# r4dl/StopThePop-Rasterization

Measured on AMD Instinct MI355X. Metric: fwd+bwd frames/sec at 1920×1080, 1M Gaussians; PSNR vs reference, higher is better.
Workload: dtype f32

## Files before the change

### stopthepop-rasterization_amd/csrc/stp_binning.hip

```cpp
#include <cstdlib>
#include <cstring>
#include <rocprim/rocprim.hpp>

#include "stp_internal.h"
#include "stp_device.h"

namespace stp {

uint32_t higher_msb(uint32_t n)
{
    uint32_t msb = sizeof(n) * 4, step = msb;
    while (step > 1) {
        step /= 2;
        if (n >> msb) msb += step; else msb -= step;
    }
    if (n >> msb) msb++;
    return msb;
}

size_t scan_temp_bytes(size_t P)
{
    size_t bytes = 0;
    (void)rocprim::inclusive_scan(nullptr, bytes, (uint32_t*)nullptr, (uint32_t*)nullptr, P, rocprim::plus<uint32_t>());
    return bytes;
}

#include <rocprim/rocprim_version.hpp>
#if ROCPRIM_VERSION_MAJOR == 4 && ROCPRIM_VERSION_MINOR == 2
#define STP_OWN_ONESWEEP 1
#else
#define STP_OWN_ONESWEEP 0
#warning "stp_binning.hip: the own onesweep driver is written against rocPRIM 4.2; with this rocPRIM the tile-bit sort uses rocprim::radix_sort_pairs (check rocprim::detail::onesweep_* against this version, then extend the #if)"
#endif
namespace {
#if STP_OWN_ONESWEEP
namespace rpd = rocprim::detail;
using OsConfig = rpd::wrapped_radix_sort_onesweep_config<rocprim::default_config, uint64_t, uint32_t>;
constexpr rpd::radix_sort_onesweep_config_params os_params()
{
    rpd::radix_sort_onesweep_config_params p = OsConfig::architecture_config<rpd::target_arch::gfx950>::params;
    p.sort.items_per_thread = 8;
#ifdef STP_OS_SORT_BLOCK
    p.sort.block_size = STP_OS_SORT_BLOCK;
#endif
#ifdef STP_OS_SORT_IPT
    p.sort.items_per_thread = STP_OS_SORT_IPT;
#endif
#ifdef STP_OS_HIST_BLOCK
    p.histogram.block_size = STP_OS_HIST_BLOCK;
#endif
#ifdef STP_OS_HIST_IPT
    p.histogram.items_per_thread = STP_OS_HIST_IPT;
#endif
    return p;
}
constexpr rpd::radix_sort_onesweep_config_params OS = os_params();
constexpr unsigned OS_RADIX = 1u << OS.radix_bits_per_place;
constexpr unsigned OS_HIST_ITEMS = OS.histogram.block_size * OS.histogram.items_per_thread;
constexpr unsigned OS_SORT_ITEMS = OS.sort.block_size * OS.sort.items_per_thread;
constexpr unsigned OS_MAX_PLACES = 4;
using OsBlockId = rpd::block_id_wrapper<unsigned int, true>;

struct OsLayout {
    uint32_t* offsets;
    unsigned int* block_ids;
    rpd::onesweep_lookback_state* lookback;
    uint32_t* offsets_tmp;
    uint64_t* keys_tmp;
    uint32_t* values_tmp;
    size_t zero_bytes, total, lookback_offset;
    uint32_t sort_blocks;
};
OsLayout os_layout(char* base, size_t R)
{
    OsLayout L{};
    auto up = [](size_t v) { return (v + 255) & ~(size_t)255; };
    L.sort_blocks = (uint32_t)((R + OS_SORT_ITEMS - 1) / OS_SORT_ITEMS);
    size_t off = 0;
    L.offsets = reinterpret_cast<uint32_t*>(base + off); off += up(sizeof(uint32_t) * OS_MAX_PLACES * OS_RADIX);
    L.block_ids = reinterpret_cast<unsigned int*>(base + off); off += up(sizeof(unsigned int) * OS_MAX_PLACES);
    L.lookback = reinterpret_cast<rpd::onesweep_lookback_state*>(base + off);
    L.lookback_offset = off;
    off += up(sizeof(rpd::onesweep_lookback_state) * OS_MAX_PLACES * OS_RADIX * (size_t)L.sort_blocks);
    L.zero_bytes = off;
    L.offsets_tmp = reinterpret_cast<uint32_t*>(base + off); off += up(sizeof(uint32_t) * OS_RADIX);
    L.keys_tmp = reinterpret_cast<uint64_t*>(base + off); off += up(sizeof(uint64_t) * R);
    L.values_tmp = reinterpret_cast<uint32_t*>(base + off); off += up(sizeof(uint32_t) * R);
    L.total = off;
    return L;
}

__global__ void __launch_bounds__(OS.histogram.block_size) os_histograms_kernel(const uint64_t* keys, uint32_t* counts, uint32_t size, uint32_t full_blocks, unsigned begin_bit, unsigned end_bit)
{
    rpd::onesweep_histograms<OS.histogram.block_size, OS.histogram.items_per_thread, OS.radix_bits_per_place, false>(
        keys, counts, size, full_blocks, rocprim::identity_decomposer{}, begin_bit, end_bit);
}
__global__ void __launch_bounds__(OS.histogram.block_size) os_scan_histograms_kernel(uint32_t* offsets)
{
    rpd::onesweep_scan_histograms<OS.histogram.block_size, OS.radix_bits_per_place>(offsets);
}
__global__ void __launch_bounds__(OS.sort.block_size) os_iteration_kernel(const uint64_t* keys_in, uint64_t* keys_out, const uint32_t* values_in, uint32_t* values_out, unsigned size,
                                                                         uint32_t* offsets_in, uint32_t* offsets_out, rpd::onesweep_lookback_state* lookback, unsigned bit,
                                                                         unsigned radix_bits, unsigned full_blocks, OsBlockId ordered_bid)
{
    rpd::onesweep_iteration<OS.sort.block_size, OS.sort.items_per_thread, OS.radix_bits_per_place, false, OS.radix_rank_algorithm>(
        keys_in, keys_out, values_in, values_out, size, offsets_in, offsets_out, lookback, rocprim::identity_decomposer{}, bit, radix_bits, full_blocks, ordered_bid);
}

constexpr uint32_t OWN_MIN = 1u << 16, OWN_MAX = 1u << 30;
bool own_onesweep_driver(size_t R)
{
    const bool lib = switches().tile_sort == Switches::TILE_SORT_ROCPRIM;
    const bool always = switches().tile_sort == Switches::TILE_SORT_OWN;
    return !lib && (R >= OWN_MIN || (always && R > 0)) && R < OWN_MAX;
}
#else
struct OsLayout { size_t total; };
OsLayout os_layout(char*, size_t) { return OsLayout{0}; }
bool own_onesweep_driver(size_t) { return false; }
#endif
}

size_t sort_temp_bytes(size_t R)
{
    size_t bytes = 0;
    (void)rocprim::radix_sort_pairs(nullptr, bytes, (uint64_t*)nullptr, (uint64_t*)nullptr, (uint32_t*)nullptr, (uint32_t*)nullptr,
                                    R, 0u, 64u);
    const size_t own = os_layout(nullptr, R).total;
    return bytes > own ? bytes : own;
}

void sort_zero_region(const BinningState& b, size_t R, uint32_t tiles, uint32_t** ptr, size_t* words)
{
    *ptr = nullptr; *words = 0;
    if (!own_onesweep_driver(R)) return;
#if STP_OWN_ONESWEEP
    const OsLayout L = os_layout(b.sort_temp, R);
    const uint32_t bit = higher_msb(tiles);
    const size_t places = (bit + OS.radix_bits_per_place - 1) / OS.radix_bits_per_place;
    const size_t bytes = L.lookback_offset + ((sizeof(rpd::onesweep_lookback_state) * places * OS_RADIX * (size_t)L.sort_blocks + 255) & ~(size_t)255);
    *ptr = reinterpret_cast<uint32_t*>(b.sort_temp);
    *words = (bytes < L.zero_bytes ? bytes : L.zero_bytes) / sizeof(uint32_t);
#else
    (void)b; (void)tiles;
#endif
}

hipError_t launch_scan(const FrameParams& f, const GeometryState& g, hipStream_t st)
{
    size_t bytes = g.scan_temp_bytes;
    return rocprim::inclusive_scan(g.scan_temp, bytes, g.tiles_touched, g.point_offsets, (size_t)f.P, rocprim::plus<uint32_t>(), st);
}

hipError_t launch_sort(const FrameParams& f, const BinningState& b, int R, bool tile_bits_only, bool zeroed, hipStream_t st)
{
    if (R <= 0) return hipSuccess;
    const uint32_t bit = higher_msb((uint32_t)(f.gx * f.gy));
    if (!(tile_bits_only && zeroed && own_onesweep_driver((size_t)R))) {
        size_t bytes = b.sort_temp_bytes;
        return rocprim::radix_sort_pairs(b.sort_temp, bytes, b.keys_unsorted, b.keys, b.point_list_unsorted, b.point_list, (size_t)R,
                                         tile_bits_only ? 32u : 0u, 32u + bit, st);
    }
#if STP_OWN_ONESWEEP
    const OsLayout L = os_layout(b.sort_temp, (size_t)R);
    const unsigned begin_bit = 32u, end_bit = 32u + bit;
    const unsigned places = (bit + OS.radix_bits_per_place - 1) / OS.radix_bits_per_place;
    const uint32_t size = (uint32_t)R;
    {
        const uint32_t blocks = (size + OS_HIST_ITEMS - 1) / OS_HIST_ITEMS, full_blocks = size % OS_HIST_ITEMS == 0 ? blocks : blocks - 1;
        hipLaunchKernelGGL(os_histograms_kernel, dim3(blocks), dim3(OS.histogram.block_size), 0, st, b.keys_unsorted, L.offsets, size, full_blocks, begin_bit, end_bit);
        hipLaunchKernelGGL(os_scan_histograms_kernel, dim3(places), dim3(OS.histogram.block_size), 0, st, L.offsets);
    }
    const uint32_t blocks = L.sort_blocks, full_blocks = size % OS_SORT_ITEMS == 0 ? blocks : blocks - 1;
    bool to_output = (places - 1) % 2 == 0, from_input = true;
    for (unsigned place = 0, pbit = begin_bit; place < places; place++, pbit += OS.radix_bits_per_place) {
        const uint64_t* kin = from_input ? b.keys_unsorted : (to_output ? L.keys_tmp : b.keys);
        const uint32_t* vin = from_input ? b.point_list_unsorted : (to_output ? L.values_tmp : b.point_list);
        uint64_t* kout = to_output ? b.keys : L.keys_tmp;
        uint32_t* vout = to_output ? b.point_list : L.values_tmp;
        const unsigned radix_bits = end_bit - pbit < OS.radix_bits_per_place ? end_bit - pbit : OS.radix_bits_per_place;
        hipLaunchKernelGGL(os_iteration_kernel, dim3(blocks), dim3(OS.sort.block_size), 0, st, kin, kout, vin, vout, size, L.offsets + place * OS_RADIX, L.offsets_tmp,
                           L.lookback + (size_t)place * OS_RADIX * blocks, pbit, radix_bits, full_blocks, OsBlockId::create(L.block_ids + place));
        from_input = false;
        to_output = !to_output;
    }
#endif
    return hipGetLastError();
}

namespace {

constexpr int SCAN_THREADS = 1024;

__global__ void __launch_bounds__(SCAN_THREADS) tile_scan_kernel(int tile0, int T, const uint32_t* __restrict__ counts_, uint2* __restrict__ ranges_,
                                                                 uint32_t* __restrict__ cursor_, uint32_t* __restrict__ total)
{
    const uint32_t* __restrict__ counts = counts_ + tile0;
    uint2* __restrict__ ranges = ranges_ + tile0;
    uint32_t* __restrict__ cursor = cursor_ + tile0;
    __shared__ uint32_t s_part[SCAN_THREADS];
    const int tid = (int)threadIdx.x;
    const int per = (T + SCAN_THREADS - 1) / SCAN_THREADS;
    const int lo = min(tid * per, T), hi = min(lo + per, T);
    uint32_t sum = 0;
    for (int t = lo; t < hi; t++) sum += counts[t];
    s_part[tid] = sum;
    __syncthreads();
    for (int off = 1; off < SCAN_THREADS; off <<= 1) {
        const uint32_t v = tid >= off ? s_part[tid - off] : 0u;
        __syncthreads();
        s_part[tid] += v;
        __syncthreads();
    }
    uint32_t run = s_part[tid] - sum;
    for (int t = lo; t < hi; t++) {
        const uint32_t c = counts[t];
        ranges[t] = c ? make_uint2(run, run + c) : make_uint2(0u, 0u);
        cursor[t] = run;
        run += c;
    }
    if (tid == SCAN_THREADS - 1) total[0] = s_part[tid];
}

__global__ void __launch_bounds__(256) bin_pad_kernel(int R, const uint32_t* __restrict__ total, uint64_t* __restrict__ keys, uint32_t* __restrict__ list)
{
    for (int i = (int)total[0] + (int)threadIdx.x; i < R; i += 256) {
        keys[i] = make_sort_key(INVALID_TILE_ID, FLT_MAX);
        list[i] = 0xFFFFFFFFu;
    }
}

}

hipError_t launch_tile_scan(const FrameParams& f, const ImageState& img, hipStream_t st)
{
    hipLaunchKernelGGL(tile_scan_kernel, dim3(1), dim3(SCAN_THREADS), 0, st, f.gx * f.ty0, f.gx * (f.ty1 - f.ty0), img.tile_counts, img.ranges, img.tile_cursor, img.bin_total);
    return hipGetLastError();
}

hipError_t launch_bin_pad(const BinningState& b, const ImageState& img, int R, hipStream_t st)
{
    if (R <= 0) return hipSuccess;
    hipLaunchKernelGGL(bin_pad_kernel, dim3(1), dim3(256), 0, st, R, img.bin_total, b.keys, b.point_list);
    return hipGetLastError();
}

}
```

### stopthepop-rasterization_amd/csrc/stp_forward.hip

```cpp
#include "stp_internal.h"

#include <atomic>
#include <cstring>
#include <mutex>
#include <string>

using namespace stp;

namespace {
struct Mailbox { volatile uint32_t* host = nullptr; uint32_t* dev = nullptr; hipEvent_t ev = nullptr; hipEvent_t done = nullptr; int device = 0; uint32_t ticket = 0; };
constexpr int MAILBOX_RING = 8;
struct MailboxRing { Mailbox slot[MAILBOX_RING]; std::atomic<unsigned> next{0}; std::atomic<bool> ready{false};
                     uint32_t* log_need = nullptr;  };
MailboxRing g_mailboxes[MAX_DEVICES];
std::mutex g_mailbox_mutex;
constexpr int GUESS_SLOTS = 16;
struct SizeGuess { std::atomic<uint64_t> key{0}; std::atomic<uint32_t> R{0}; std::atomic<uint32_t> log_need{0}; };
SizeGuess g_guess[MAX_DEVICES][GUESS_SLOTS];
uint64_t guess_key(const FrameParams& f)
{
    uint64_t k = 0x9E3779B97F4A7C15ull;
    for (uint64_t v : {(uint64_t)f.P, (uint64_t)f.W, (uint64_t)f.H, (uint64_t)f.ty0, (uint64_t)f.ty1, (uint64_t)f.s.sort_mode,
                       (uint64_t)(f.s.tile_based_culling * 8 + f.s.rect_bounding * 4 + f.s.tight_opacity_bounding * 2 + (f.s.sort_order == ORDER_PTD_MAX))})
        k = (k ^ v) * 0xBF58476D1CE4E5B9ull, k ^= k >> 29;
// ... 84 lines not shown
    SideStream* side = nullptr;
    bool colour_started = true;
    char* bin_ptr = nullptr; size_t bin_have = 0;
    uint32_t cap = 0; bool ahead = false, run_ahead = false;
    int* radii; float* const out_color;
    struct Split { const ForwardSplit s; hipStream_t st; bool recorded; ~Split() { if (s.armed && !recorded) (void)hipEventRecord(s.event, st); } } split;
    SideJoin colours;

    ForwardCall(hipStream_t stream, int debug_, const ForwardSplit& split_, int* radii_, float* out_color_)
        : st(stream), debug(debug_), radii(radii_), out_color(out_color_), split{split_, stream, false}, colours{nullptr, stream, false} {}
    int carve_geometry_and_image(stp_alloc_fn geometry_alloc, void* geometry_user, stp_alloc_fn image_alloc, void* image_user, bool with_inv, bool with_stash);
    int launch_up_to_mailbox(); int colour_on_side();
    int request_binning(stp_alloc_fn binning_alloc, void* binning_user);
    int wait_mailbox(); int read_mailbox(int* R_out, bool* wild_out);
    int binning_and_render(const GeometryState& gd, const BinningState& b, int L, uint32_t dup_cap);
};

int ForwardCall::carve_geometry_and_image(stp_alloc_fn geometry_alloc, void* geometry_user, stp_alloc_fn image_alloc, void* image_user, bool with_inv, bool with_stash)
{
    size_t geom_bytes = 0;
    carve_geometry(nullptr, (size_t)f.P, with_inv, &geom_bytes, nullptr, nullptr, with_stash ? &sh_stash : nullptr);
    char* geom_ptr = (char*)geometry_alloc(geometry_user, geom_bytes);
    if (!geom_ptr) return fail(STP_ERR_ALLOC, "geometry allocator returned NULL");
    g = carve_geometry(geom_ptr, (size_t)f.P, with_inv, nullptr, nullptr, nullptr, with_stash ? &sh_stash : nullptr);
    geom_base = geom_ptr;
    if (!radii) radii = g.internal_radii;

    if (int rc = acquire_mailbox(&mb)) return rc;
    colours.done = mb.done;
    gkey = guess_key(f);
    const unsigned gidx = (unsigned)((gkey >> 1) % GUESS_SLOTS);
    gslot = &g_guess[mb.device][gidx];
    log_need_word = g_mailboxes[mb.device].log_need + gidx;
    size_t img_bytes = 0;
    with_log = uses_blend_log(f.s);
    log_depth = with_log ? log_depth_for(*gslot, gkey) : 0;
    f.log_depth = log_depth;
    f.log_need = with_log ? log_need_word : nullptr;
    log_tag = (uint32_t)((gkey >> 40) & 0xFFFFu) | 1u;
    f.log_tag = log_tag;
    carve_image(nullptr, f.W, f.H, f.ty0, f.ty1, log_depth, &img_bytes);
    img_ptr = (char*)image_alloc(image_user, img_bytes);
    if (!img_ptr) return fail(STP_ERR_ALLOC, "image allocator returned NULL");
    img = carve_image(img_ptr, f.W, f.H, f.ty0, f.ty1, log_depth, nullptr);
    return 0;
}

int ForwardCall::launch_up_to_mailbox()
{
    const bool atomic_bin = switches().atomic_bin, two_level_scan = switches().two_level_scan;
    timer_begin_forward();
    timer_mark(0, st);
    STP_TRY(launch_frame_init(g, img, f.gx * f.ty0, f.gx * (f.ty1 - f.ty0), with_log, atomic_bin, st), "frame init launch");
    STP_TRY(launch_preprocess(f, g, radii, atomic_bin ? img.tile_counts : nullptr, st), "preprocess launch");
    STP_DEBUG_SYNC("preprocess");
    if (!two_level_scan) STP_TRY(launch_scan(f, g, st), "inclusive scan");
    STP_DEBUG_SYNC("scan");
    if (atomic_bin) STP_TRY(launch_tile_scan(f, img, st), "tile scan");

    if (two_level_scan) STP_TRY(launch_block_prefix_mailbox(f, g, mb.dev, mb.ticket, log_need_word, st), "workgroup prefixes + mailbox launch");
    else STP_TRY(launch_mailbox(g.point_offsets + (f.P - 1), g.status + 1, mb.dev, mb.ticket, log_need_word, st), "mailbox launch");
    STP_TRY(hipEventRecord(mb.ev, st), "record mailbox event");
    side = side_stream(mb.device);
    colour_started = !(side && switches().colour_late);
    if (side) {
        if (colour_started) { if (int rc = colour_on_side()) return rc; }
    } else STP_TRY(launch_sh_color(f, g, radii, sh_stash, st), "SH colour launch");
    return 0;
}

int ForwardCall::colour_on_side()
{
    STP_TRY(hipStreamWaitEvent(side->stream, mb.ev, 0), "side stream wait");
    STP_TRY(launch_sh_color(f, g, radii, sh_stash, side->stream), "SH colour launch");
    if (hipError_t e = hipEventRecord(mb.done, side->stream); e != hipSuccess) {
        (void)hipStreamSynchronize(side->stream);
        return fail_hip(e, "record colour event");
    }
    colours.pending = true;
    return 0;
}

int ForwardCall::request_binning(stp_alloc_fn binning_alloc, void* binning_user)
{
    const Switches& sw = switches();
    const int run_ahead_mode = g_run_ahead.load(std::memory_order_relaxed);
    run_ahead = run_ahead_mode != 0;
    const uint32_t guess = (sw.speculative_binning && gslot->key.load(std::memory_order_acquire) == gkey) ? gslot->R.load(std::memory_order_relaxed) : 0u;
    ahead = run_ahead && guess > 0 && (run_ahead_mode == 1 || guess < RUN_AHEAD_AUTO_MAX) && sw.two_level_scan && !sw.atomic_bin && !debug;
    cap = guess + guess / 8 + (ahead ? 1024u : 0u);
    if (guess > 0) {
        carve_binning(nullptr, (size_t)cap, &bin_have);
        bin_ptr = (char*)binning_alloc(binning_user, bin_have);
        if (!bin_ptr) return fail(STP_ERR_ALLOC, "binning allocator returned NULL");
    }
    return 0;
}

int ForwardCall::wait_mailbox()
{
    const bool mbx_spin = switches().mailbox_spin;
    if (mbx_spin) {
        for (unsigned it = 1;; it++) {
            if (mb.host[2] == mb.ticket) break;
            if ((it & 255u) == 0u) {
                const hipError_t q = hipEventQuery(mb.ev);
                if (q == hipSuccess) break;
                if (q != hipErrorNotReady) return fail_hip(q, "query (num_rendered)");
                if (it > (1u << 22)) { STP_TRY(hipEventSynchronize(mb.ev), "synchronize (num_rendered)"); break; }
            }
            cpu_relax();
        }
        std::atomic_thread_fence(std::memory_order_acquire);
    } else STP_TRY(hipEventSynchronize(mb.ev), "synchronize (num_rendered)");
    return 0;
}

int ForwardCall::read_mailbox(int* R_out, bool* wild_out)
{
    if (int rc = wait_mailbox()) return rc;
    const uint32_t host_status[2] = {mb.host[0], mb.host[1]};
    const uint32_t word = mb.host[3];
    if (const uint32_t reported = (word >> 16) == log_tag ? (word & 0xFFFFu) : 0u) {
        const uint32_t known = gslot->key.load(std::memory_order_acquire) == gkey ? gslot->log_need.load(std::memory_order_relaxed) : 0u;
        const uint32_t keep = known - known / 32;
        gslot->log_need.store(reported > keep ? reported : keep, std::memory_order_relaxed);
    } else if (gslot->key.load(std::memory_order_acquire) != gkey) gslot->log_need.store(0u, std::memory_order_relaxed);
    if (host_status[1] & 1u) return fail(STP_ERR_PREFILTERED, "Point is filtered although prefiltered is set. This shouldn't happen!");
    *wild_out = (host_status[1] & 2u) != 0;
    *R_out = (int)host_status[0];
    const uint32_t prev = gslot->key.load(std::memory_order_acquire) == gkey ? gslot->R.load(std::memory_order_relaxed) : 0u;
    const uint32_t keep = run_ahead ? prev - prev / 32 : 0u;
    gslot->R.store((uint32_t)*R_out > keep ? (uint32_t)*R_out : keep, std::memory_order_relaxed);
    gslot->key.store(gkey, std::memory_order_release);
    return 0;
}

int ForwardCall::binning_and_render(const GeometryState& gd, const BinningState& b, int L, uint32_t dup_cap)
{
    const bool atomic_bin = switches().atomic_bin, tile_local_sort = switches().tile_local_sort;
    uint32_t* zero_ptr = nullptr; size_t zero_words = 0;
    if (!atomic_bin && tile_local_sort) sort_zero_region(b, (size_t)L, (uint32_t)(f.gx * f.gy), &zero_ptr, &zero_words);
    STP_TRY(launch_duplicate(f, gd, radii, b, atomic_bin ? img.tile_cursor : nullptr, dup_cap, (uint32_t)L, zero_ptr, zero_words, st), "duplicate launch");
    STP_DEBUG_SYNC("duplicate");
    timer_mark(2, st);
    if (!colour_started) {
        STP_TRY(hipEventRecord(mb.ev, st), "record event behind duplicate");
        if (int rc = colour_on_side()) return rc;
        colour_started = true;
    }
    if (atomic_bin) {
        STP_TRY(launch_bin_pad(b, img, L, st), "pad entries");
    } else {
        STP_TRY(launch_sort(f, b, L, tile_local_sort, zero_words != 0, st), "radix sort");
        STP_DEBUG_SYNC("sort");
        STP_TRY(launch_ranges(f, b, img, L, st), "tile ranges");
        STP_DEBUG_SYNC("ranges");
    }
    const bool order_wanted = !atomic_bin && tile_order_used(f);
#ifdef STP_ORDER_MAIN
    const bool order_on_side = false;
#else
    const bool order_on_side = order_wanted && side != nullptr && gather_order_mode() == 0 && f.gx * (f.ty1 - f.ty0) >= 16384;
#endif
    if (order_on_side) {
        STP_TRY(hipEventRecord(mb.ev, st), "record event behind the ranges");
        STP_TRY(hipStreamWaitEvent(side->stream, mb.ev, 0), "side stream wait (ranges)");
        STP_TRY(launch_tile_order(f, img, side->stream), "tile order");
    } else if (order_wanted) STP_TRY(launch_tile_order(f, img, st), "tile order");
    STP_TRY(colours.join(), "join colour stream");
    SideJoin ordering{mb.done, st, false};
    if (order_on_side) {
        if (hipError_t e = hipEventRecord(mb.done, side->stream); e != hipSuccess) {
            (void)hipStreamSynchronize(side->stream);
            return fail_hip(e, "record tile-order event");
        }
        ordering.pending = true;
    }
    if (tile_local_sort) STP_TRY(launch_tile_sort_gather(f, g, b, img, L, atomic_bin, st), "tile sort + entry gather");
    else STP_TRY(launch_gather_entries(f, g, b, L, st), "entry gather");
    STP_DEBUG_SYNC("entry gather");
    STP_TRY(ordering.join(), "join tile order");
    timer_mark(3, st);
    std::string err;
    hipError_t e;
    if (split.s.armed && split.s.row > f.ty0 && split.s.row < f.ty1 && f.s.debug_visualization == 0) {
        FrameParams f1 = f, f2 = f;
        f1.ty1 = split.s.row; f2.ty0 = split.s.row;
        f1.split_launch = f2.split_launch = 1;
        e = launch_render_forward(f1, g, b, img, out_color, st, &err);
        if (e == hipSuccess) { e = hipEventRecord(split.s.event, st); split.recorded = e == hipSuccess; }
        if (e == hipSuccess) e = launch_render_forward(f2, g, b, img, out_color, st, &err);
    } else e = launch_render_forward(f, g, b, img, out_color, st, &err);
    if (e != hipSuccess) {
        if (!err.empty()) return fail(STP_ERR_QUEUE_SIZE, err);
        return fail_hip(e, "render launch");
    }
    STP_DEBUG_SYNC("render");
    STP_TRY(launch_render_debug_finish(f, img, out_color, st), "debug visualisation");
    timer_mark(4, st);
    return 0;
}
}

extern "C" {

void stp_set_run_ahead(int mode) { g_run_ahead.store(mode < 0 ? 0 : (mode > 2 ? 2 : mode), std::memory_order_relaxed); }
int stp_get_run_ahead(void) { return g_run_ahead.load(std::memory_order_relaxed); }
void stp_reset_size_guesses(void)
{
    for (auto& dev : g_guess)
        for (auto& slot : dev) { slot.key.store(0, std::memory_order_release); slot.R.store(0u, std::memory_order_relaxed); slot.log_need.store(0u, std::memory_order_relaxed); }
    int cur = 0;
    if (hipGetDevice(&cur) != hipSuccess) return;
    for (int d = 0; d < MAX_DEVICES; d++)
        if (g_mailboxes[d].ready.load(std::memory_order_acquire) && g_mailboxes[d].log_need && hipSetDevice(d) == hipSuccess) {
            (void)hipDeviceSynchronize();
            (void)hipMemset(g_mailboxes[d].log_need, 0, sizeof(uint32_t) * 64);
        }
    (void)hipSetDevice(cur);
}

int stp_forward(stp_alloc_fn geometry_alloc, void* geometry_user, stp_alloc_fn binning_alloc, void* binning_user,
                stp_alloc_fn image_alloc, void* image_user, int P, int D, int M, const float* background, int width, int height,
                const StpSettings* settings, const float* means3D, const float* shs, const float* colors_precomp,
                const float* opacities, const float* scales, float scale_modifier, const float* rotations,
                const float* cov3D_precomp, const float* viewmatrix, const float* projmatrix, const float* inv_viewprojmatrix,
                const float* cam_pos, float tan_fovx, float tan_fovy, int prefiltered, float* out_color, int* radii, int debug,
                void* stream)
{
    const ForwardRequests req = take_forward_requests();
    ForwardCall c((hipStream_t)stream, debug, req.split, radii, out_color);
    const ForwardBackground& fbg = req.background;
    if (!settings || !geometry_alloc || !binning_alloc || !image_alloc) return fail(STP_ERR_INVALID_ARGUMENT, "null settings or allocator");
    if (P < 0 || width <= 0 || height <= 0) return fail(STP_ERR_INVALID_ARGUMENT, "bad sizes");
    if (P == 0) return 0;
    if (!means3D || !opacities || !background || !viewmatrix || !projmatrix || !inv_viewprojmatrix || !cam_pos || !out_color)
        return fail(STP_ERR_INVALID_ARGUMENT, "null required input");
    if (int rc = check_settings(*settings, false)) return rc;
    if ((fbg.bg_image || fbg.out_alpha) && settings->debug_visualization == STP_DEBUG_DEPTH)
        return fail(STP_ERR_INVALID_ARGUMENT, "alpha output / per-pixel background (stp_set_forward_background) are not available with the debug depth visualisation: its image is not C + T * background");
    if (req.out_invdepth && settings->debug_visualization == STP_DEBUG_DEPTH)
        return fail(STP_ERR_INVALID_ARGUMENT, "the inverse-depth output (stp_set_forward_invdepth) is not available with the debug depth visualisation");
    if (int rc = check_raw_params(req.raw_params, opacities, scales, rotations)) return rc;
    const float* const sh_dc = colors_precomp ? nullptr : req.sh_dc;
    if (sh_dc && M > 1 && !shs) return fail(STP_ERR_INVALID_ARGUMENT, "split SH (stp_set_forward_split_sh): M > 1 needs the rest of the coefficients in shs");
    if (!colors_precomp && !shs && !sh_dc) return fail(STP_ERR_INVALID_ARGUMENT, "neither SHs nor precomputed colours given");
    if (!cov3D_precomp && !(scales && rotations)) return fail(STP_ERR_INVALID_ARGUMENT, "neither scale/rotation nor precomputed covariance given");
    const bool with_inv = requires_depth_along_ray(*settings);
    if (with_inv && !(scales && rotations)) return fail(STP_ERR_NEEDS_SCALE_ROTATION, "sorted modes need scales and rotations");

    FrameParams& f = c.f;
    fill_frame(f, P, D, M, background, width, height, *settings, means3D, shs, colors_precomp, opacities, scales, scale_modifier,
               rotations, cov3D_precomp, viewmatrix, projmatrix, inv_viewprojmatrix, cam_pos, tan_fovx, tan_fovy, prefiltered);
    f.out_invdepth = req.out_invdepth;
    f.sh_dc = sh_dc;
    f.raw_params = req.raw_params;
    f.bg_image = fbg.bg_image; f.out_alpha = fbg.out_alpha;
    const bool with_stash = req.sh_stash && !colors_precomp && (shs || sh_dc) && M > 0;
    if (int rc = c.carve_geometry_and_image(geometry_alloc, geometry_user, image_alloc, image_user, with_inv, with_stash)) return rc;

    const Switches& sw = switches();
    f.fused_gather = sw.fused_gather && sw.tile_local_sort && !sw.atomic_bin && f.s.sort_mode == MODE_HIER && f.s.debug_visualization != STP_DEBUG_DEPTH ? 1 : 0;
    if (!sw.two_level_scan) { c.g.block_sums = nullptr; c.g.block_prefix = nullptr; }

    if (int rc = c.launch_up_to_mailbox()) return rc;
    if (int rc = c.request_binning(binning_alloc, binning_user)) return rc;

    const hipStream_t st = c.st;
    int R = 0;
    bool wild = false;
    GeometryState g_dup = c.g;
    if (c.ahead) {
        f.wild_cov = 0;
        timer_mark(1, st);
        const BinningState b = carve_binning(c.bin_ptr, (size_t)c.cap, nullptr);
        if (int rc = c.binning_and_render(g_dup, b, (int)c.cap, c.cap)) return rc;
        if (int rc = c.read_mailbox(&R, &wild)) return rc;
        if ((uint32_t)R <= c.cap && !wild) {
            remember_stash(c.geom_base, with_stash, R);
            remember_layout(c.bin_ptr, c.cap, R);
            remember_log_depth(c.img_ptr, (uint32_t)c.log_depth, R);
            return R;
        }
        g_dup.block_prefix = nullptr; g_dup.block_sums = nullptr;
        STP_TRY(launch_frame_init(c.g, c.img, f.gx * f.ty0, f.gx * (f.ty1 - f.ty0), c.with_log, sw.atomic_bin, st), "frame init launch");
        STP_TRY(launch_stash_mark(f, c.g, c.sh_stash, st), "stash mark launch");
    } else {
        if (int rc = c.read_mailbox(&R, &wild)) return rc;
        STP_DEBUG_SYNC("SH colour");
        timer_mark(1, st);
    }
    f.wild_cov = wild ? 1 : 0;
    size_t bin_bytes = 0;
    carve_binning(nullptr, (size_t)R, &bin_bytes);
    if (bin_bytes > c.bin_have) {
        c.bin_ptr = (char*)binning_alloc(binning_user, bin_bytes);
        if (!c.bin_ptr) return fail(STP_ERR_ALLOC, "binning allocator returned NULL");
    }
    const BinningState b = carve_binning(c.bin_ptr, (size_t)R, nullptr);
    if (int rc = c.binning_and_render(g_dup, b, R, 0xFFFFFFFFu)) return rc;
    remember_stash(c.geom_base, with_stash, R);
    if (c.bin_ptr) remember_layout(c.bin_ptr, (uint32_t)R, R);
    remember_log_depth(c.img_ptr, (uint32_t)c.log_depth, R);
    return R;
}
}
```

### stopthepop-rasterization_amd/csrc/stp_internal.h

```cpp
#pragma once

#include <hip/hip_runtime.h>
#include <cstdint>
#include <cstddef>
#include <cstdlib>
#include <string>

#include "../../include/stp_raster.h"
#include "stp_switches.h"

namespace stp {

constexpr int TILE = 16;
constexpr size_t ALIGN = 256;
static_assert(ALIGN == 256, "Switches::carve_skew (stp_switches.h) is masked to a multiple of 256");
constexpr int MAX_DEVICES = 32;

enum SortMode { MODE_GLOBAL = 0, MODE_FULL = 1, MODE_KBUFFER = 2, MODE_HIER = 3 };
enum SortOrder { ORDER_Z = 0, ORDER_DISTANCE = 1, ORDER_PTD_CENTER = 2, ORDER_PTD_MAX = 3 };

inline bool uses_blend_log(const StpSettings& s)
{
    return s.record_blend_log != 0 && s.debug_visualization == 0 && (s.sort_mode == MODE_HIER || s.sort_mode == MODE_KBUFFER);
}
// ... 51 lines not shown

struct ImageState {
    float* final_T;
    uint32_t* n_contrib;
    uint2* ranges;
    uint32_t* dbg_minmax;
    uint32_t* tile_counts;
    uint32_t* tile_cursor;
    uint32_t* bin_total;
    uint32_t* header;
    uint32_t* tile_flags;
    uint32_t* blend_log;
    int log_depth;
};

struct BinningState {
    uint32_t* header;
    uint32_t* point_list;
    uint32_t* point_list_unsorted;
    uint64_t* keys;
    uint64_t* keys_unsorted;
    char* sort_temp;
    size_t sort_temp_bytes;
    float4* entA;
    float4* entB;
    float4* entC;
    float4* entD;
    float4* entF;
};

constexpr uint32_t STP_HEADER_MAGIC_BINNING = 0x42505453u, STP_HEADER_MAGIC_IMAGE = 0x49505453u;
struct NamedOffset { const char* name; size_t offset; size_t count; };

GeometryState carve_geometry(char* base, size_t P, bool with_inv, size_t* total, NamedOffset* names = nullptr, int* n_names = nullptr, float** sh_stash = nullptr);
ImageState carve_image(char* base, int W, int H, int ty0, int ty1, int log_depth , size_t* total, NamedOffset* names = nullptr, int* n_names = nullptr);
BinningState carve_binning(char* base, size_t R, size_t* total, NamedOffset* names = nullptr, int* n_names = nullptr);
void clamp_tile_rows(int height, int& y0, int& y1);

int fail(int code, const std::string& msg);
int fail_hip(hipError_t e, const char* what);
#define STP_TRY(expr, what) do { hipError_t _e = (expr); if (_e != hipSuccess) return fail_hip(_e, what); } while (0)
#define STP_DEBUG_SYNC(what)  STP_TRY(debug ? hipStreamSynchronize(st) : hipSuccess, what)

void timer_begin_forward();
void timer_begin_backward();
void timer_mark(int i, hipStream_t st);

void remember_layout(const void* binning, uint32_t count, int64_t R);
void remember_stash(const void* geometry, bool stash, int64_t R);
int stash_of(const char* geometry, int P, int64_t R, bool* stash, hipStream_t st, bool have_stream);
void remember_log_depth(const void* image, uint32_t depth, int64_t R);
int layout_of(const char* binning, uint32_t R, uint32_t* cap, hipStream_t st = nullptr, bool have_stream = false);
int log_depth_of(const char* image, int64_t R, uint32_t* depth, hipStream_t st = nullptr, bool have_stream = false);

int blend_log_rows(int depth);
int blend_log_default_depth();
int blend_log_clamp_depth(int d);
size_t scan_temp_bytes(size_t P);
size_t sort_temp_bytes(size_t R);

struct FrameParams {
    int P, D, M, W, H, gx, gy;
    int ty0, ty1;
    float focal_x, focal_y, tan_fovx, tan_fovy, scale_modifier;
    StpSettings s;
    const float* background;
    const float* means3D;
    const float* shs;
    const float* colors_precomp;
    const float* opacities;
    const float* scales;
    const float* rotations;
    const float* cov3D_precomp;
    const float* viewmatrix;
    const float* projmatrix;
    const float* inv_viewprojmatrix;
    const float* cam_pos;
    int prefiltered;
    int log_depth;
    uint32_t* log_need;
    uint32_t log_tag;
    int split_launch = 0;
    int fused_gather = 0;
    const float* bg_image = nullptr;
    float* out_alpha = nullptr;
    float* out_invdepth = nullptr;
    const float* sh_dc = nullptr;
    int raw_params = 0;
    int wild_cov;
};

struct CameraGradRequest {
    float* dL_dview = nullptr;
    float* dL_dproj = nullptr;
    float* dL_dcam = nullptr;
    void* workspace = nullptr;
    size_t workspace_bytes = 0;
};

struct BackwardParams {
    CameraGradRequest cam;
    float* absgrad = nullptr;
    float* blend_stats = nullptr;
    const float* bg_image = nullptr;
    const float* dL_dalpha = nullptr;
    float* dL_dbackground = nullptr;
    const float* invdepth = nullptr;
    const float* dL_dinvdepth = nullptr;
    const float* pixel_colors;
    const float* dL_dpix;
    float* grad_rec;
    int grad_stride;
    int clear_rec;
    int chunk, chunks;
    float* dL_dmean2D;
    float* dL_dopacity;
    float* dL_dcolor;
    float* dL_dmean3D;
    float* dL_dcov3D;
    float* dL_dsh;
    float* dL_dscale;
    float* dL_drot;
    const float* sh_stash = nullptr;
    float* dL_ddc = nullptr;
};

int check_settings(const StpSettings& s, bool backward);
void fill_frame(FrameParams& f, int P, int D, int M, const float* background, int width, int height, const StpSettings& s, const float* means3D,
                const float* shs, const float* colors_precomp, const float* opacities, const float* scales, float scale_modifier, const float* rotations,
                const float* cov3D_precomp, const float* viewmatrix, const float* projmatrix, const float* inv_viewprojmatrix, const float* cam_pos,
                float tan_fovx, float tan_fovy, int prefiltered);

struct ForwardSplit { int row = 0; hipEvent_t event = nullptr; bool armed = false; };
struct ForwardBackground { const float* bg_image = nullptr; float* out_alpha = nullptr; };
struct ForwardRequests { ForwardSplit split; ForwardBackground background; float* out_invdepth = nullptr;  const float* sh_dc = nullptr;  bool sh_stash = false;  int raw_params = 0;  };
ForwardRequests take_forward_requests();
int check_raw_params(int mask, const float* opacities, const float* scales, const float* rotations);

hipError_t launch_preprocess(const FrameParams& f, const GeometryState& g, int* radii, uint32_t* tile_counts, hipStream_t st);
hipError_t launch_frame_init(const GeometryState& g, const ImageState& img, int tile0, int n_tiles, bool with_log, bool tile_counters, hipStream_t st);
hipError_t launch_scan(const FrameParams& f, const GeometryState& g, hipStream_t st);
bool tile_order_enabled();
inline bool tile_order_used(const FrameParams& f) { return tile_order_enabled() && f.gx * (f.ty1 - f.ty0) > 1024; }
bool gather_order_enabled();
int gather_order_mode();
hipError_t launch_tile_order(const FrameParams& f, const ImageState& img, hipStream_t st);
hipError_t launch_sh_color(const FrameParams& f, const GeometryState& g, const int* radii, float* sh_stash, hipStream_t st);
hipError_t launch_stash_mark(const FrameParams& f, const GeometryState& g, float* sh_stash, hipStream_t st);
hipError_t launch_mailbox(const uint32_t* last_offset, const uint32_t* status, uint32_t* mailbox_dev, uint32_t ticket, uint32_t* log_need, hipStream_t st);
hipError_t launch_block_prefix_mailbox(const FrameParams& f, const GeometryState& g, uint32_t* mailbox_dev, uint32_t ticket, uint32_t* log_need, hipStream_t st);
hipError_t launch_duplicate(const FrameParams& f, const GeometryState& g, const int* radii, const BinningState& b, uint32_t* tile_cursor, uint32_t cap, uint32_t header_cap, uint32_t* zero_ptr, size_t zero_words, hipStream_t st);
hipError_t launch_tile_scan(const FrameParams& f, const ImageState& img, hipStream_t st);
hipError_t launch_bin_pad(const BinningState& b, const ImageState& img, int R, hipStream_t st);
hipError_t launch_sort(const FrameParams& f, const BinningState& b, int R, bool tile_bits_only, bool zeroed, hipStream_t st);
void sort_zero_region(const BinningState& b, size_t R, uint32_t tiles, uint32_t** ptr, size_t* words);
hipError_t launch_tile_sort_gather(const FrameParams& f, const GeometryState& g, const BinningState& b, const ImageState& img, int R, bool unordered, hipStream_t st);
hipError_t launch_ranges(const FrameParams& f, const BinningState& b, const ImageState& img, int R, hipStream_t st);
hipError_t launch_gather_entries(const FrameParams& f, const GeometryState& g, const BinningState& b, int R, hipStream_t st);
hipError_t launch_render_forward(const FrameParams& f, const GeometryState& g, const BinningState& b, const ImageState& img,
                                 float* out_color, hipStream_t st, std::string* err);
hipError_t launch_render_debug_finish(const FrameParams& f, const ImageState& img, float* out_color, hipStream_t st);
hipError_t launch_render_backward(const FrameParams& f, const GeometryState& g, const BinningState& b, const ImageState& img,
                                  const BackwardParams& bw, hipStream_t st, std::string* err);
size_t background_grad_partials();
hipError_t launch_background_grad(const FrameParams& f, const ImageState& img, const BackwardParams& bw, float* partials, hipStream_t st);
hipError_t launch_preprocess_backward(const FrameParams& f, const GeometryState& g, const int* radii, const BackwardParams& bw, hipStream_t st);
size_t camera_grad_workspace_bytes(int P);
hipError_t launch_camera_grad_finalize(int P, const CameraGradRequest& cam, hipStream_t st);
hipError_t launch_mark_visible(int P, const float* means3D, const float* viewmatrix, uint8_t* present, hipStream_t st);
int launch_sparse_adam(int n_tensors, const StpAdamTensor* tensors, int N, const void* visible, int visible_kind, float beta1, float beta2,
                       hipStream_t st, hipError_t* err);
int launch_activate_params(int P, const float* scaling, const float* rotation, const float* opacity, float* scales, float* rotations, float* opacities,
                           hipStream_t st, hipError_t* err);
int launch_mcmc_relocation(int n, const float* opacity_old, const float* scale_old, const void* N, int n_kind, int n_max, float* opacity_new,
                           float* scale_new, hipStream_t st, hipError_t* err);
int launch_mcmc_add_noise(int P, float* xyz, const float* scales, const float* rotations, const float* opacities, const float* noise, float noise_scale,
                          float k, float x0, int raw, hipStream_t st, hipError_t* err);
size_t mcmc_relocate_scratch_bytes(int P);
int launch_mcmc_sample(int P, const float* opacity, int rule, float min_opacity, int raw, int n_draws, const float* uniforms, void* scratch, uint32_t* weights,
                       int32_t* src, int32_t* count, hipStream_t st, hipError_t* err);
int launch_mcmc_relocate_apply(int P, const int32_t* src, const int32_t* count, int n_tensors, const StpMcmcTensor* tensors, float min_opacity, int raw,
                               int reset_dead_moments, void* scratch, hipStream_t st, hipError_t* err);
int launch_mcmc_add_apply(int P, int n_new, const int32_t* src, const int32_t* count, int n_tensors, const StpMcmcTensor* tensors, float min_opacity, int raw,
                          void* scratch, hipStream_t st, hipError_t* err);
int launch_densify_stats(int P, float* grad_accum, float* denom, float* max_radii2D, const float* grad2d, int grad_stride, const void* visible,
                         int visible_kind, hipStream_t st, hipError_t* err);
int launch_densify_plan(int P, const float* grad_accum, const float* denom, const float* scaling, const float* opacity, const float* max_radii2D,
                        const StpDensifyRule& rule, uint8_t* plan, hipStream_t st, hipError_t* err);
size_t densify_scratch_bytes(int P);
int launch_densify_scan(int P, const uint8_t* plan, void* scratch, uint32_t* offsets, int64_t counts[3], hipStream_t st, hipError_t* err);
int launch_densify_apply(int P, const uint8_t* plan, const uint32_t* offsets, const int64_t counts[3], int n_tensors, const StpDensifyTensor* tensors,
                         const float* noise, float split_shrink, int raw, hipStream_t st, hipError_t* err);
uint32_t photometric_groups(int planes, int H, int W);
int launch_photometric_forward(int planes, int H, int W, const float* image, const float* target, float* out2, float* maps, float* workspace,
                               hipStream_t st, hipError_t* err);
int launch_photometric_backward(int planes, int H, int W, const float* image, const float* target, const float* maps, const float* dL_dout2,
                                float* dL_dimage, hipStream_t st, hipError_t* err);

size_t knn_scratch_bytes(int P);
int launch_knn_mean_dist2(int P, const float* points, void* scratch, float* mean_dist2, hipStream_t st, hipError_t* err);

uint32_t higher_msb(uint32_t n);

}
```

### stopthepop-rasterization_amd/csrc/stp_switches.h

```cpp
#pragma once
#include <cstddef>
#include <cstdlib>
#include <cstring>

namespace stp {

struct Switches {
    bool tile_local_sort;
    bool atomic_bin;
    bool fused_gather;
    bool two_level_scan;
    bool colour_late;
    bool speculative_binning;
    bool mailbox_spin;
    bool side_stream;
    int fixed_log_depth;
    size_t carve_skew;
    bool tile_order;
    int gather_order;
    enum TileSort { TILE_SORT_AUTO, TILE_SORT_ROCPRIM, TILE_SORT_OWN } tile_sort;
    enum KBuffer { KBUFFER_RING, KBUFFER_TILE, KBUFFER_WAVE } kbuffer;
};

inline const Switches& switches()
{
    static const Switches table = [] {
        const auto is = [](const char* name, const char* value) { const char* e = std::getenv(name); return e && std::strcmp(e, value) == 0; };
        const auto starts_with_0 = [](const char* name) { const char* e = std::getenv(name); return e && e[0] == '0'; };
        const auto number = [](const char* name) { const char* e = std::getenv(name); return e ? std::atoi(e) : 0; };
        Switches s{};
        s.tile_local_sort = !is("STP_SORT", "radix");
        s.atomic_bin = is("STP_SORT", "counters");
        s.fused_gather = !starts_with_0("STP_FUSED_GATHER");
        s.two_level_scan = !is("STP_SCAN", "rocprim");
        s.colour_late = !starts_with_0("STP_COLOUR_LATE");
        s.speculative_binning = !is("STP_BINNING", "exact");
        s.mailbox_spin = !is("STP_MAILBOX", "event");
        s.side_stream = !is("STP_SIDE_STREAM", "0");
        s.fixed_log_depth = number("STP_LOG_DEPTH");
        const char* skew = std::getenv("STP_CARVE_SKEW");
        s.carve_skew = skew ? ((size_t)std::strtoull(skew, nullptr, 0) & ~(size_t)255) : (size_t)0;
        s.tile_order = !starts_with_0("STP_TILE_ORDER");
        s.gather_order = number("STP_GATHER_ORDER");
        s.tile_sort = is("STP_TILE_SORT", "rocprim") ? Switches::TILE_SORT_ROCPRIM : is("STP_TILE_SORT", "own") ? Switches::TILE_SORT_OWN : Switches::TILE_SORT_AUTO;
        s.kbuffer = is("STP_KBUFFER", "tile") ? Switches::KBUFFER_TILE : is("STP_KBUFFER", "wave") ? Switches::KBUFFER_WAVE : Switches::KBUFFER_RING;
        return s;
    }();
    return table;
}

}
```

Measured before the change: 460.6.

## Replace final onesweep passes with LDS bucket-finish sort that also emits tile ranges

When the tile-key bit count is small, the onesweep radix sort now runs only one pass on the top radix digit. A new two-kernel bucket finish then sorts the remaining low bits inside each bucket in shared memory, splitting large buckets into parts with a count kernel. The scatter kernel also writes the per-tile ranges directly, so the separate ranges kernel is skipped. This is meant to save a full global radix pass and the ranges pass, at the cost of new, more complex kernels, large dynamic LDS use and extra scratch for part totals.

```diff
diff --git a/stopthepop-rasterization_amd/csrc/stp_binning.hip b/stopthepop-rasterization_amd/csrc/stp_binning.hip
--- a/stopthepop-rasterization_amd/csrc/stp_binning.hip
+++ b/stopthepop-rasterization_amd/csrc/stp_binning.hip
@@ -68,6 +68,7 @@
     uint32_t* offsets_tmp;
     uint64_t* keys_tmp;
     uint32_t* values_tmp;
+    uint32_t* part_totals;
     size_t zero_bytes, total, lookback_offset;
     uint32_t sort_blocks;
 };
@@ -86,6 +87,7 @@
     L.offsets_tmp = reinterpret_cast<uint32_t*>(base + off); off += up(sizeof(uint32_t) * OS_RADIX);
     L.keys_tmp = reinterpret_cast<uint64_t*>(base + off); off += up(sizeof(uint64_t) * R);
     L.values_tmp = reinterpret_cast<uint32_t*>(base + off); off += up(sizeof(uint32_t) * R);
+    L.part_totals = reinterpret_cast<uint32_t*>(base + off); off += up(sizeof(uint32_t) * bucket_finish_scratch_words(R));
     L.total = off;
     return L;
 }
@@ -108,6 +110,8 @@
 }
 
 constexpr uint32_t OWN_MIN = 1u << 16, OWN_MAX = 1u << 30;
+constexpr uint32_t BUCKET_FINISH_MAX_BIT = 13;
+bool bucket_finish_path(uint32_t bit) { return switches().bucket_finish && bit > OS.radix_bits_per_place && bit <= BUCKET_FINISH_MAX_BIT; }
 bool own_onesweep_driver(size_t R)
 {
     const bool lib = switches().tile_sort == Switches::TILE_SORT_ROCPRIM;
@@ -137,7 +141,7 @@
 #if STP_OWN_ONESWEEP
     const OsLayout L = os_layout(b.sort_temp, R);
     const uint32_t bit = higher_msb(tiles);
-    const size_t places = (bit + OS.radix_bits_per_place - 1) / OS.radix_bits_per_place;
+    const size_t places = bucket_finish_path(bit) ? 1 : (bit + OS.radix_bits_per_place - 1) / OS.radix_bits_per_place;
     const size_t bytes = L.lookback_offset + ((sizeof(rpd::onesweep_lookback_state) * places * OS_RADIX * (size_t)L.sort_blocks + 255) & ~(size_t)255);
     *ptr = reinterpret_cast<uint32_t*>(b.sort_temp);
     *words = (bytes < L.zero_bytes ? bytes : L.zero_bytes) / sizeof(uint32_t);
@@ -152,8 +156,9 @@
     return rocprim::inclusive_scan(g.scan_temp, bytes, g.tiles_touched, g.point_offsets, (size_t)f.P, rocprim::plus<uint32_t>(), st);
 }
 
-hipError_t launch_sort(const FrameParams& f, const BinningState& b, int R, bool tile_bits_only, bool zeroed, hipStream_t st)
-{
+hipError_t launch_sort(const FrameParams& f, const BinningState& b, int R, bool tile_bits_only, bool zeroed, uint2* ranges, bool* ranges_done, hipStream_t st)
+{
+    *ranges_done = false;
     if (R <= 0) return hipSuccess;
     const uint32_t bit = higher_msb((uint32_t)(f.gx * f.gy));
     if (!(tile_bits_only && zeroed && own_onesweep_driver((size_t)R))) {
@@ -163,8 +168,9 @@
     }
 #if STP_OWN_ONESWEEP
     const OsLayout L = os_layout(b.sort_temp, (size_t)R);
-    const unsigned begin_bit = 32u, end_bit = 32u + bit;
-    const unsigned places = (bit + OS.radix_bits_per_place - 1) / OS.radix_bits_per_place;
+    const bool finish = ranges != nullptr && bucket_finish_path(bit);
+    const unsigned end_bit = 32u + bit, begin_bit = finish ? end_bit - OS.radix_bits_per_place : 32u;
+    const unsigned places = finish ? 1u : (bit + OS.radix_bits_per_place - 1) / OS.radix_bits_per_place;
     const uint32_t size = (uint32_t)R;
     {
         const uint32_t blocks = (size + OS_HIST_ITEMS - 1) / OS_HIST_ITEMS, full_blocks = size % OS_HIST_ITEMS == 0 ? blocks : blocks - 1;
@@ -172,7 +178,7 @@
         hipLaunchKernelGGL(os_scan_histograms_kernel, dim3(places), dim3(OS.histogram.block_size), 0, st, L.offsets);
     }
     const uint32_t blocks = L.sort_blocks, full_blocks = size % OS_SORT_ITEMS == 0 ? blocks : blocks - 1;
-    bool to_output = (places - 1) % 2 == 0, from_input = true;
+    bool to_output = !finish && (places - 1) % 2 == 0, from_input = true;
     for (unsigned place = 0, pbit = begin_bit; place < places; place++, pbit += OS.radix_bits_per_place) {
         const uint64_t* kin = from_input ? b.keys_unsorted : (to_output ? L.keys_tmp : b.keys);
         const uint32_t* vin = from_input ? b.point_list_unsorted : (to_output ? L.values_tmp : b.point_list);
@@ -183,6 +189,12 @@
                            L.lookback + (size_t)place * OS_RADIX * blocks, pbit, radix_bits, full_blocks, OsBlockId::create(L.block_ids + place));
         from_input = false;
         to_output = !to_output;
+    }
+    if (finish) {
+        if (hipError_t e = hipGetLastError(); e != hipSuccess) return e;
+        *ranges_done = true;
+        return launch_bucket_finish(L.keys_tmp, L.values_tmp, b.keys, b.point_list, size, L.offsets, bit - OS.radix_bits_per_place, L.part_totals, ranges,
+                                    (uint32_t)(f.gx * f.gy), st);
     }
 #endif
     return hipGetLastError();
diff --git a/stopthepop-rasterization_amd/csrc/stp_bucket_sort.hip b/stopthepop-rasterization_amd/csrc/stp_bucket_sort.hip
--- /dev/null
+++ b/stopthepop-rasterization_amd/csrc/stp_bucket_sort.hip
@@ -0,0 +1,252 @@
+#include "stp_internal.h"
+#include "stp_device.h"
+
+namespace stp {
+namespace {
+
+constexpr int BF_THREADS = 1024, BF_WAVES = BF_THREADS / 64, BF_BINS = 256, BF_BUCKETS = 256, BF_UNROLL = 4;
+constexpr unsigned BF_LOW_BITS_MAX = 5;
+constexpr int BF_ITEMS = 16;
+constexpr uint32_t BF_PART_MAX = BF_THREADS * BF_ITEMS;
+
+struct BfArgs {
+    const uint64_t* keys_in;
+    const uint32_t* values_in;
+    uint64_t* keys_out;
+    uint32_t* values_out;
+    const uint32_t* bucket_offsets;
+    uint32_t* part_totals;
+    uint2* ranges;
+    uint32_t R, part, rows, T;
+    unsigned low_bits;
+};
+
+struct BfWork { uint32_t bucket, part, nparts, first_row, start, size; };
+
+__device__ __forceinline__ unsigned long long lanes_lt() { return (1ull << lane_id()) - 1ull; }
+
+__device__ __forceinline__ uint32_t scan256_inclusive(uint32_t v, uint32_t* s_wave, int tid)
+{
+    const int lane = tid & 63, wave = tid >> 6;
+#pragma unroll
+    for (int d = 1; d < 64; d <<= 1) {
+        const uint32_t t = (uint32_t)__shfl_up((int)v, d);
+        if (lane >= d) v += t;
+    }
+    if (lane == 63 && wave < 4) s_wave[wave] = v;
+    __syncthreads();
+    for (int k = 0; k < wave && k < 4; k++) v += s_wave[k];
+    __syncthreads();
+    return v;
+}
+
+__device__ __forceinline__ bool bf_locate(const BfArgs& a, uint32_t row, uint32_t* s_wave, BfWork* s_work, int tid)
+{
+    uint32_t start = 0, size = 0, np = 0;
+    if (tid < BF_BUCKETS) {
+        start = min(a.bucket_offsets[tid], a.R);
+        const uint32_t next = tid + 1 < BF_BUCKETS ? min(a.bucket_offsets[tid + 1], a.R) : a.R;
+        size = next > start ? next - start : 0u;
+        np = (size + a.part - 1) / a.part;
+    }
+    if (tid == 0) s_work->nparts = 0u;
+    const uint32_t incl = scan256_inclusive(np, s_wave, tid);
+    if (tid < BF_BUCKETS && row >= incl - np && row < incl) {
+        s_work->bucket = (uint32_t)tid; s_work->part = row - (incl - np); s_work->nparts = np;
+        s_work->first_row = incl - np; s_work->start = start; s_work->size = size;
+    }
+    __syncthreads();
+    return s_work->nparts != 0u;
+}
+
+__device__ __forceinline__ unsigned long long bf_peers(bool valid, uint32_t d, unsigned low_bits)
+{
+    unsigned long long peers = __ballot(valid);
+    for (unsigned bit = 0; bit < low_bits; bit++) {
+        const bool one = ((d >> bit) & 1u) != 0u;
+        const unsigned long long bal = __ballot(one);
+        peers &= one ? bal : ~bal;
+    }
+    return peers;
+}
+
+__device__ __forceinline__ void bf_count_slice(const BfArgs& a, uint32_t lo, uint32_t hi, uint32_t* s_row)
+{
+    const uint32_t* __restrict__ tiles = reinterpret_cast<const uint32_t*>(a.keys_in);
+    const uint32_t mask = (1u << a.low_bits) - 1u, lane = (uint32_t)lane_id();
+    const unsigned long long lt = lanes_lt();
+    for (uint32_t i0 = lo; i0 < hi; i0 += 64u * BF_UNROLL) {
+        uint32_t d[BF_UNROLL];
+#pragma unroll
+        for (int r = 0; r < BF_UNROLL; r++) {
+            const uint32_t i = i0 + 64u * r + lane;
+            d[r] = i < hi ? tiles[2 * (size_t)i + 1] & mask : 0u;
+        }
+#pragma unroll
+        for (int r = 0; r < BF_UNROLL; r++) {
+            const bool valid = i0 + 64u * r + lane < hi;
+            const unsigned long long peers = bf_peers(valid, d[r], a.low_bits);
+            if (valid && (peers & lt) == 0ull) s_row[d[r]] += (uint32_t)__popcll(peers);
+            wave_sync();
+        }
+    }
+}
+
+__device__ __forceinline__ void bf_slice(const BfWork& w, uint32_t part_size, int wave, uint32_t& lo, uint32_t& hi)
+{
+    const uint32_t p0 = w.part * part_size, n = min(part_size, w.size - p0);
+    const uint32_t slice = ((n + BF_WAVES - 1) / BF_WAVES + 63u) & ~63u;
+    lo = min((uint32_t)wave * slice, n); hi = min(lo + slice, n);
+    lo += w.start + p0; hi += w.start + p0;
+}
+
+__global__ void __launch_bounds__(BF_THREADS) bucket_count_kernel(const BfArgs a)
+{
+    __shared__ uint32_t s_cnt[BF_WAVES][BF_BINS];
+    __shared__ uint32_t s_wave[4];
+    __shared__ BfWork s_work;
+    const int tid = (int)threadIdx.x, wave = tid >> 6;
+    if (!bf_locate(a, blockIdx.x, s_wave, &s_work, tid)) return;
+    const BfWork w = s_work;
+    if (w.nparts < 2u) return;
+    for (int i = tid; i < BF_WAVES * BF_BINS; i += BF_THREADS) (&s_cnt[0][0])[i] = 0u;
+    __syncthreads();
+    uint32_t lo, hi;
+    bf_slice(w, a.part, wave, lo, hi);
+    bf_count_slice(a, lo, hi, s_cnt[wave]);
+    __syncthreads();
+    if (tid < BF_BINS && blockIdx.x < a.rows) {
+        uint32_t total = 0;
+        for (int k = 0; k < BF_WAVES; k++) total += s_cnt[k][tid];
+        a.part_totals[(size_t)blockIdx.x * BF_BINS + tid] = total;
+    }
+}
+
+template <unsigned LOW_BITS> __global__ void __launch_bounds__(BF_THREADS) bucket_scatter_kernel(const BfArgs a)
+{
+    extern __shared__ uint2 s_data[];
+    __shared__ uint32_t s_cnt[BF_WAVES][BF_BINS];
+    __shared__ uint32_t s_own[BF_BINS], s_lstart[BF_BINS], s_gbase[BF_BINS], s_hi[BF_BINS];
+    __shared__ uint32_t s_wave[4];
+    __shared__ BfWork s_work;
+    const int tid = (int)threadIdx.x, wave = tid >> 6, lane = tid & 63;
+    if (!bf_locate(a, blockIdx.x, s_wave, &s_work, tid)) return;
+    const BfWork w = s_work;
+    uint32_t lo, hi;
+    bf_slice(w, a.part, wave, lo, hi);
+
+    const uint32_t* __restrict__ words = reinterpret_cast<const uint32_t*>(a.keys_in);
+    uint32_t* const s_row = s_cnt[wave];
+    uint32_t pk[BF_ITEMS];
+#pragma unroll
+    for (int r = 0; r < BF_ITEMS; r++) {
+        const uint32_t i = lo + 64u * r + (uint32_t)lane;
+        pk[r] = i < hi ? words[2 * (size_t)i + 1] : 0u;
+    }
+#pragma unroll
+    for (int k = 0; k < BF_BINS / 64; k++) s_row[64 * k + lane] = 0u;
+    wave_sync();
+    constexpr uint32_t mask = (1u << LOW_BITS) - 1u;
+    const unsigned long long lt = lanes_lt();
+#pragma unroll
+    for (int r = 0; r < BF_ITEMS; r++) {
+        if (lo + 64u * r < hi) {
+            const bool valid = lo + 64u * r + (uint32_t)lane < hi;
+            const uint32_t d = pk[r] & mask;
+            unsigned long long peers = __ballot(valid);
+#pragma unroll
+            for (unsigned bit = 0; bit < LOW_BITS; bit++) {
+                const bool one = ((d >> bit) & 1u) != 0u;
+                const unsigned long long bal = __ballot(one);
+                peers &= one ? bal : ~bal;
+            }
+            const uint32_t rank = (uint32_t)__popcll(peers & lt), seen = s_row[d];
+            wave_sync();
+            if (valid && rank == 0u) {
+                s_row[d] = seen + (uint32_t)__popcll(peers);
+                s_hi[d] = pk[r];
+            }
+            wave_sync();
+            pk[r] = (d << 16) | (seen + rank);
+        }
+    }
+    __syncthreads();
+
+    uint32_t own = 0, total = 0, earlier = 0;
+    if (tid < BF_BINS) {
+        for (int k = 0; k < BF_WAVES; k++) own += s_cnt[k][tid];
+        total = own;
+        if (w.nparts > 1u) {
+            total = 0;
+            const uint32_t rows = w.first_row < a.rows ? min(w.nparts, a.rows - w.first_row) : 0u;
+            for (uint32_t q = 0; q < rows; q++) {
+                const uint32_t c = a.part_totals[(size_t)(w.first_row + q) * BF_BINS + tid];
+                total += c;
+                if (q < w.part) earlier += c;
+            }
+        }
+    }
+    const uint32_t before = scan256_inclusive(total, s_wave, tid) - total;
+    const uint32_t lstart = scan256_inclusive(own, s_wave, tid) - own;
+    if (tid < BF_BINS) {
+        const uint32_t first = w.start + before;
+        uint32_t run = lstart;
+        for (int k = 0; k < BF_WAVES; k++) { const uint32_t c = s_cnt[k][tid]; s_cnt[k][tid] = run; run += c; }
+        s_own[tid] = own; s_lstart[tid] = lstart; s_gbase[tid] = first + earlier;
+        const uint32_t tile = (w.bucket << LOW_BITS) | (uint32_t)tid;
+        if (w.part == 0u && total > 0u && (uint32_t)tid <= mask && tile < a.T) a.ranges[tile] = make_uint2(min(first, a.R), min(first + total, a.R));
+    }
+    __syncthreads();
+#pragma unroll
+    for (int r = 0; r < BF_ITEMS; r++) {
+        const uint32_t i = lo + 64u * r + (uint32_t)lane;
+        if (i < hi) {
+            const uint32_t at = s_row[pk[r] >> 16] + (pk[r] & 0xFFFFu);
+            if (at < a.part) s_data[at] = make_uint2(words[2 * (size_t)i], a.values_in[i]);
+        }
+    }
+    __syncthreads();
+    constexpr int NB = 1 << LOW_BITS, G = NB >= BF_WAVES ? 1 : BF_WAVES / NB;
+    for (int b = wave / G; b < NB; b += BF_WAVES / G) {
+        const uint32_t n = min(s_own[b], a.part), ls = s_lstart[b], gb = s_gbase[b];
+        const uint64_t tile_word = (uint64_t)s_hi[b] << 32;
+        for (uint32_t k = (uint32_t)((wave % G) * 64 + lane); k < n; k += 64u * G) {
+            const uint32_t dst = gb + k;
+            if (ls + k < a.part && dst < a.R) {
+                const uint2 e = s_data[ls + k];
+                a.keys_out[dst] = tile_word | e.x;
+                a.values_out[dst] = e.y;
+            }
+        }
+    }
+}
+
+}
+
+size_t bucket_finish_scratch_words(size_t R)
+{
+    const size_t part = switches().bucket_part;
+    return ((R + part - 1) / part + BF_BUCKETS) * BF_BINS;
+}
+
+hipError_t launch_bucket_finish(const uint64_t* keys_in, const uint32_t* values_in, uint64_t* keys_out, uint32_t* values_out, uint32_t R, const uint32_t* bucket_offsets,
+                                unsigned low_bits, uint32_t* part_totals, uint2* ranges, uint32_t T, hipStream_t st)
+{
+    if (R == 0u) return hipSuccess;
+    if (low_bits < 1u || low_bits > BF_LOW_BITS_MAX) return hipErrorInvalidValue;
+    BfArgs a;
+    a.keys_in = keys_in; a.values_in = values_in; a.keys_out = keys_out; a.values_out = values_out;
+    a.bucket_offsets = bucket_offsets; a.part_totals = part_totals; a.ranges = ranges;
+    a.R = R; a.part = switches().bucket_part;
+    if (a.part > BF_PART_MAX || a.part % (64u * BF_WAVES) != 0u) return hipErrorInvalidValue; a.T = T; a.low_bits = low_bits;
+    a.rows = (uint32_t)(bucket_finish_scratch_words(R) / BF_BINS);
+    if (R > a.part) hipLaunchKernelGGL(bucket_count_kernel, dim3(a.rows), dim3(BF_THREADS), 0, st, a);
+    using Kernel = void (*)(const BfArgs);
+    static const Kernel scatter[BF_LOW_BITS_MAX] = {bucket_scatter_kernel<1>, bucket_scatter_kernel<2>, bucket_scatter_kernel<3>, bucket_scatter_kernel<4>, bucket_scatter_kernel<5>};
+    const size_t lds = (size_t)a.part * sizeof(uint2);
+    if (hipError_t e = hipFuncSetAttribute(reinterpret_cast<const void*>(scatter[low_bits - 1u]), hipFuncAttributeMaxDynamicSharedMemorySize, (int)lds); e != hipSuccess) return e;
+    hipLaunchKernelGGL(scatter[low_bits - 1u], dim3(a.rows), dim3(BF_THREADS), lds, st, a);
+    return hipGetLastError();
+}
+
+}
diff --git a/stopthepop-rasterization_amd/csrc/stp_forward.hip b/stopthepop-rasterization_amd/csrc/stp_forward.hip
--- a/stopthepop-rasterization_amd/csrc/stp_forward.hip
+++ b/stopthepop-rasterization_amd/csrc/stp_forward.hip
@@ -260,9 +260,10 @@
     if (atomic_bin) {
         STP_TRY(launch_bin_pad(b, img, L, st), "pad entries");
     } else {
-        STP_TRY(launch_sort(f, b, L, tile_local_sort, zero_words != 0, st), "radix sort");
+        bool ranges_done = false;
+        STP_TRY(launch_sort(f, b, L, tile_local_sort, zero_words != 0, img.ranges, &ranges_done, st), "radix sort");
         STP_DEBUG_SYNC("sort");
-        STP_TRY(launch_ranges(f, b, img, L, st), "tile ranges");
+        if (!ranges_done) STP_TRY(launch_ranges(f, b, img, L, st), "tile ranges");
         STP_DEBUG_SYNC("ranges");
     }
     const bool order_wanted = !atomic_bin && tile_order_used(f);
diff --git a/stopthepop-rasterization_amd/csrc/stp_internal.h b/stopthepop-rasterization_amd/csrc/stp_internal.h
--- a/stopthepop-rasterization_amd/csrc/stp_internal.h
+++ b/stopthepop-rasterization_amd/csrc/stp_internal.h
@@ -227,7 +227,10 @@
 hipError_t launch_duplicate(const FrameParams& f, const GeometryState& g, const int* radii, const BinningState& b, uint32_t* tile_cursor, uint32_t cap, uint32_t header_cap, uint32_t* zero_ptr, size_t zero_words, hipStream_t st);
 hipError_t launch_tile_scan(const FrameParams& f, const ImageState& img, hipStream_t st);
 hipError_t launch_bin_pad(const BinningState& b, const ImageState& img, int R, hipStream_t st);
-hipError_t launch_sort(const FrameParams& f, const BinningState& b, int R, bool tile_bits_only, bool zeroed, hipStream_t st);
+hipError_t launch_sort(const FrameParams& f, const BinningState& b, int R, bool tile_bits_only, bool zeroed, uint2* ranges, bool* ranges_done, hipStream_t st);
+size_t bucket_finish_scratch_words(size_t R);
+hipError_t launch_bucket_finish(const uint64_t* keys_in, const uint32_t* values_in, uint64_t* keys_out, uint32_t* values_out, uint32_t R, const uint32_t* bucket_offsets,
+                                unsigned low_bits, uint32_t* part_totals, uint2* ranges, uint32_t T, hipStream_t st);
 void sort_zero_region(const BinningState& b, size_t R, uint32_t tiles, uint32_t** ptr, size_t* words);
 hipError_t launch_tile_sort_gather(const FrameParams& f, const GeometryState& g, const BinningState& b, const ImageState& img, int R, bool unordered, hipStream_t st);
 hipError_t launch_ranges(const FrameParams& f, const BinningState& b, const ImageState& img, int R, hipStream_t st);
diff --git a/stopthepop-rasterization_amd/csrc/stp_switches.h b/stopthepop-rasterization_amd/csrc/stp_switches.h
--- a/stopthepop-rasterization_amd/csrc/stp_switches.h
+++ b/stopthepop-rasterization_amd/csrc/stp_switches.h
@@ -18,6 +18,8 @@
     size_t carve_skew;
     bool tile_order;
     int gather_order;
+    bool bucket_finish;
+    unsigned bucket_part;
     enum TileSort { TILE_SORT_AUTO, TILE_SORT_ROCPRIM, TILE_SORT_OWN } tile_sort;
     enum KBuffer { KBUFFER_RING, KBUFFER_TILE, KBUFFER_WAVE } kbuffer;
 };
@@ -42,6 +44,9 @@
         s.carve_skew = skew ? ((size_t)std::strtoull(skew, nullptr, 0) & ~(size_t)255) : (size_t)0;
         s.tile_order = !starts_with_0("STP_TILE_ORDER");
         s.gather_order = number("STP_GATHER_ORDER");
+        s.bucket_finish = !is("STP_TILE_BITS", "onesweep");
+        const int part = number("STP_BUCKET_PART");
+        s.bucket_part = part <= 0 ? 16384u : (unsigned)(part < 1024 ? 1024 : part > 16384 ? 16384 : part / 1024 * 1024);
         s.tile_sort = is("STP_TILE_SORT", "rocprim") ? Switches::TILE_SORT_ROCPRIM : is("STP_TILE_SORT", "own") ? Switches::TILE_SORT_OWN : Switches::TILE_SORT_AUTO;
         s.kbuffer = is("STP_KBUFFER", "tile") ? Switches::KBUFFER_TILE : is("STP_KBUFFER", "wave") ? Switches::KBUFFER_WAVE : Switches::KBUFFER_RING;
         return s;
```

Result: no change. 463.7 (median of 6 runs) (+0.7%).
